# HKUST-KnowComp/DummyNode4GraphLearning

Hardware: AMD Instinct MI355X
Metric: edges/sec fwd+bwd on dummy-augmented RGIN conv (higher is better)
Workload: dtype bf16; 1 GPU; config5: RGINLayer(256,256,R=16,basis,relu) fwd+bwd, ONE global batch of 32768 graphs cut by parallel.shard_graphs over 1 GPU(s) (rank 0: N=1015808, E=3997696), SI dummy augmentation; global_edges=3997696, parallelism=dp1, rows_P=3112960, grad_bucket_bytes=2491904, hip_graph=True, sub_batches=1

## Files before the change

dummynode4graphlearning_amd/_lib.py:

```python
import ctypes
import os

import torch

_HERE = os.path.dirname(os.path.abspath(__file__))
LIB_PATH = os.environ.get("DN_HIP_LIB") or os.path.join(_HERE, "libdn_hip.so")

c_i32, c_i64, c_f32, c_sz = ctypes.c_int32, ctypes.c_int64, ctypes.c_float, ctypes.c_size_t
P = ctypes.c_void_p

class WgradJob(ctypes.Structure):
    _fields_ = [("A", P), ("A2", P), ("idx_a", P), ("G", P), ("G2", P), ("idx_g", P), ("mask_a_bits", P), ("na1", c_i32), ("ng1", c_i32),
                ("colsum_of", c_i32), ("first_rel", c_i32), ("row0", c_i32), ("act_slope", c_f32)]


class BatchCol(ctypes.Structure):
    _fields_ = [("src", P), ("dst", P), ("row_bytes", c_i32), ("level", c_i32), ("rebase", c_i32), ("int_width", c_i32),
                ("src_global", c_i32), ("ptr_tail", c_i32)]


_SIGS = {
    "dn_version": (ctypes.c_int, []),
    "dn_last_error": (ctypes.c_char_p, []),
    "dn_runtime_probe": (ctypes.c_int, [P]),
# ... 41 lines not shown
                                                P, P, P]),
    "dn_layer_graphs_bwd_bf16": (ctypes.c_int, [P, c_i32, P, P, c_i32, P, P, c_f32, P, P, P, P, P, P, P, c_i64, c_i64, P, P, P, P, P, P, P,
                                                P]),
    "dn_conv_graphs_max_nodes": (c_i32, []),
    "dn_conv_graphs_max_edges": (c_i32, []),
    "dn_conv_graphs_bf16": (ctypes.c_int, [P, c_i32, P, c_i32, P, P, c_i32, P, P, P, P, P, c_i64, c_i64, P, P, P, P, P, P]),
    "dn_conv_index_workspace_bytes": (c_sz, [c_i64, c_i64, c_i64, c_i64, c_i32, c_i64]),
    "dn_conv_index_build_i32": (ctypes.c_int, [c_i64, c_i64, c_i64, c_i64, P, P, P, P, P, c_i32, c_f32] + [P] * 10 +
                                [ctypes.POINTER(c_i64), ctypes.POINTER(c_i32), ctypes.POINTER(c_i32),
                                 ctypes.POINTER(c_i32), P, P, P, P, P, ctypes.POINTER(c_i32)] +
                                [c_i32, c_i32, c_i64] + [P] * 8 + [c_i32, c_i64] + [P] * 8 + [c_i32, c_i32, P, P] + [c_i32, c_i32, c_i64, P, P] +
                                [ctypes.POINTER(c_i32), P, c_sz, P]),
    "dn_row_tables_build_i32": (ctypes.c_int, [c_i32, P, c_i32, c_i64, P, P, ctypes.c_uint64, P]),
    "dn_sweep_tables_build_i32": (ctypes.c_int, [c_i32, P, P, P, c_i64, c_i32, c_i32, ctypes.c_uint64, P, P, P]),
    "dn_slot_table_build_i32": (ctypes.c_int, [c_i64, c_i32, c_i32, P, P, c_i32, c_i32, P, P, P, P]),
    "dn_fold_tables_build_async_i32": (ctypes.c_int, [c_i64, c_i64, P, P, P, P, P, P, c_sz, P]),
    "dn_rows_wgrad_workspace_bytes": (c_sz, [c_i64, c_i32, c_i32]),
    "dn_rows_wgrad_bf16": (ctypes.c_int, [P, P, c_i32, P, P, P, c_i32, P, c_i32, c_i32, c_i64, P, c_i64, P, P, c_i32,
                                          c_i32, P, P, P, P, P, c_f32, P, c_sz, P]),
    "dn_rows_transform_bf16": (ctypes.c_int, [P, P, c_i32, P, c_i32, c_i32, P, P, c_i32, P, P, c_i64, P, c_i32, c_f32, P]),
    "dn_relu_bwd_bf16": (ctypes.c_int, [P, P, P, c_i64, c_f32, P]),
    "dn_rows_chain2_bf16": (ctypes.c_int, [P, c_i32, P, P, c_i32, P, P, P, P, c_i32, c_i64, P, P, P, P, c_i32, c_f32, P]),
    "dn_mlp_bwd_fused_bf16": (ctypes.c_int, [P, P, P, P, P, c_i64, c_i32, P, c_i64, P, P, c_i32, P, P, P, c_f32, P, c_sz, P]),
    "dn_rows_selfsum_bf16": (ctypes.c_int, [P, c_i32, P, P, P, P, c_i32, P, c_i32, c_i64, P, P, P, c_i32, P, P, c_i32, c_i32, c_i32, P]),
    "dn_overflow_rows_add_bf16": (ctypes.c_int, [P, c_i32, P, c_i32, c_i64, P, P, c_i32, c_i32, c_i32, P, P]),
    "dn_close_units_capacity": (c_i64, [c_i64, c_i64, c_i32]),
    "dn_close_units_workspace_bytes": (c_sz, [c_i64, c_i32]),
    "dn_close_units_build_i32": (ctypes.c_int, [c_i64, c_i32, c_i32, P, c_i64, c_i32, c_i32, P, P, c_i64, c_i32, c_i32, P, P, P, c_i64, P,
                                                P, P, P, c_i32, P, c_sz, P]),
    "dn_fold_graph_tiles_build_i32": (ctypes.c_int, [c_i64, c_i64, P, P, P, P, P, P, P]),
    "dn_fold_graph_tiles_multi_capacity": (c_i64, [c_i64, c_i32]),
    "dn_fold_graph_tiles_multi_build_i32": (ctypes.c_int, [c_i64, c_i64, P, P, P, c_i32, P, P, P, P, c_i64, P, P]),
    "dn_rows_close_bf16": (ctypes.c_int, [P, c_i32, P, c_i32, P, P, P, P, c_i32, P, P, c_i64, P, P, P, P, P, P, P]),
    "dn_bdd_compose": (ctypes.c_int, [P, c_i64, c_i32, c_i32, c_i32, c_i32, P, P]),
    "dn_bdd_extract": (ctypes.c_int, [P, c_i64, c_i32, c_i32, c_i32, c_i32, P, P]),
    "dn_fold_tables_workspace_bytes": (c_sz, [c_i64]),
    "dn_fold_tables_build_i32": (ctypes.c_int, [c_i64, c_i64, P, P, P, P, ctypes.POINTER(ctypes.c_int32), P, c_sz, P]),
    "dn_fold_tail_bf16": (ctypes.c_int, [P, P, c_i64, c_i32, P, P, P, P, c_i32, P]),
    "dn_rows_transform_f32": (ctypes.c_int, [P, P, c_i32, P, c_i32, c_i32, P, P, c_i32, P, P, c_i64, P, c_i32, c_f32, P, c_i32, c_i32, c_i32, P]),
    "dn_rows_wgrad_f32": (ctypes.c_int, [P, P, c_i32, P, P, P, c_i32, P, c_i32, c_i32, c_i64, P, c_i64, P, P, c_i32, P, P, P,
                                         c_i32, c_f32, P, c_sz, P]),
    "dn_relu_bwd_f32": (ctypes.c_int, [P, P, P, c_i64, c_f32, P]),
    "dn_rows_gemm_f32": (ctypes.c_int, [P, P, P, c_i32, c_i32, c_i32, P, c_i64, P, P]),
    "dn_rows_gemm_bf16": (ctypes.c_int, [P, P, P, c_i32, c_i32, c_i32, P, c_i64, P, P]),
    "dn_rows_wgrad_any_workspace_bytes": (c_sz, [c_i64, c_i32, c_i32]),
    "dn_rows_wgrad_any_f32": (ctypes.c_int, [P, P, c_i32, c_i32, c_i64, P, c_i64, P, P, P, P, c_sz, P]),
# ... 138 lines not shown
```

dummynode4graphlearning_amd/csrc/build.py:

```python
import hashlib
import os
import subprocess
import sys
from concurrent.futures import ThreadPoolExecutor

HERE = os.path.dirname(os.path.abspath(__file__))
PKG = os.path.dirname(HERE)
ROOT = os.path.dirname(PKG)
SOURCES = ["dn_runtime.hip", "dn_segment.hip", "dn_index.hip", "dn_index_local.hip", "dn_conv_index.hip", "dn_graphsum.hip", "dn_rel.hip", "dn_rel_ring.hip", "dn_close.hip", "dn_conv_graph.hip", "dn_chain2.hip", "dn_mlp_bwd.hip", "dn_weights.hip", "dn_rel_f32.hip", "dn_gemm.hip", "dn_norm.hip", "dn_simodel.hip", "dn_dual.hip", "dn_batch.hip", "dn_lrp.hip", "dn_hgt.hip"]
HEADERS = ["dn_common.h", "dn_internal.h", os.path.join(ROOT, "include", "dn_hip.h")]
LIB = os.path.join(PKG, "libdn_hip.so")
OBJDIR = os.path.join(HERE, "_obj")
ARCH = "gfx950"
FLAGS = ["-O3", "-std=c++17", "-fPIC", "--offload-arch=" + ARCH, "-fno-gpu-rdc", "-Wno-unused-result",
         "-I" + os.path.join(ROOT, "include")]


def _hipcc():
    for c in (os.environ.get("HIPCC"), "/opt/rocm/bin/hipcc", "hipcc"):
        if c and (os.path.isabs(c) and os.path.exists(c) or not os.path.isabs(c)):
            return c
    raise RuntimeError("hipcc not found")


def _digest(paths):
    h = hashlib.sha256()
    for p in paths:
        with open(p, "rb") as f:
            h.update(f.read())
    h.update(" ".join(FLAGS).encode())
    return h.hexdigest()

# ... 47 lines not shown
```

dummynode4graphlearning_amd/csrc/dn_internal.h:

```cpp
#pragma once
#include <hip/hip_runtime.h>
#include <stdint.h>

namespace dn_internal {

int launch_transform_ring256(const void* X, const void* X2, int32_t n1, const int32_t* idx, const void* Wn, const void* bias,
                             int32_t relu, int32_t nt_store, const void* mask_pos, const int32_t* tiles, int64_t num_tiles,
                             int64_t tiles_per_wg, void* Y, int32_t w_kn, float slope, hipStream_t st);

bool chain2_ring_supported(bool has_mask0, bool has_mask1, bool has_bits1, bool has_bits2);
int launch_chain2_ring256(const void* X, const void* W1n, const void* b1, const void* W2n, const void* b2, int32_t flags,
                          const void* mask0, const void* mask1, int64_t N, void* Y1, void* Y2, void* bits1, void* bits2,
                          float slope, hipStream_t st);

int launch_wgrad_reduce(const float* workspace, const int32_t* chunk_ptr, int64_t num_chunks, int32_t H, int64_t R, void* out,
                        int32_t out_is_f32, bool with_colsum, float* out_colsum, void* out_colsum_lp, hipStream_t st);

constexpr int kRilPlanWords = 14;

int ril_queue(int64_t G, int64_t N, int64_t R, int64_t E, const int32_t* node_ptr, const int32_t* edge_ptr, const int32_t* src,
              const int32_t* dst, const int32_t* etype, int32_t self_loop, float edge_frac, int32_t* row_in, int32_t* row_out,
              int32_t* aux_f_ptr, int32_t* aux_f_idx, int32_t* aux_b_ptr, int32_t* aux_b_idx, int32_t* dst_ptr, int32_t* dst_rows,
              int32_t* src_ptr, int32_t* src_rows, int32_t* rel_ptr_dev, int32_t* tile_ptr_f, int32_t* fold_info_f,
              int32_t* tile_ptr_b, int32_t* fold_info_b, bool verdicts, bool plan, void* workspace, size_t workspace_bytes,
              int32_t** meta_dev, hipStream_t st);
void ril_unpack(const int32_t* h_meta, int64_t R, int64_t* host_counts, int32_t* host_rel_ptr, int32_t* host_modes,
                int32_t* host_status, int32_t* host_absorb);

struct CloseUnitsDir {
    const int32_t *tile_ptr, *list_ptr, *list_rows;
    int32_t num_edge_rows, drop_beg, drop_end;
// ... 24 lines not shown
```

dummynode4graphlearning_amd/csrc/dn_rel_ring.hip:

```cpp
#include "dn_common.h"
#include "dn_internal.h"

namespace {

typedef __bf16 bf16_t;
typedef bf16_t bf16x8 __attribute__((ext_vector_type(8)));
typedef float f32x4 __attribute__((ext_vector_type(4)));
typedef unsigned int u32x4 __attribute__((ext_vector_type(4)));

struct Tile {
    int32_t rel, beg, end, pad;
};

constexpr int kH = 256;
constexpr int kRowB = 2 * kH;
constexpr int kTR = 32;
constexpr int kStageB = kTR * kRowB;
constexpr int kNS = 8;
constexpr int kCompute = 8, kLoaders = 4;
constexpr int kThreads = 64 * (kCompute + kLoaders);
constexpr int kRowsPerLoader = kTR / kLoaders;
constexpr int kDmaPerTile = kRowsPerLoader / 2;
constexpr int kBatch = 8;
constexpr int kRecRing = 32, kIdxRing = 16, kDescRing = 32;

__device__ __forceinline__ uint32_t pack_bf16x2(float a, float b) {
    typedef bf16_t bf16x2 __attribute__((ext_vector_type(2)));
    bf16x2 v;
    v[0] = (bf16_t)a;
    v[1] = (bf16_t)b;
    return __builtin_bit_cast(uint32_t, v);
}

#ifdef DN_RING_STATS
__device__ unsigned long long g_ring_stats[256][10];
#define DN_STAMP() __builtin_amdgcn_s_memtime()
#define DN_STAT(var, expr) var += (expr)
#else
#define DN_STAMP() 0ull
#define DN_STAT(var, expr)
#endif

__device__ int32_t g_zero_idx[64];

#define DN_DS_READ128(dst, addr, OFF) asm volatile("ds_read_b128 %0, %1 offset:" #OFF : "=v"(dst) : "v"(addr))

template <bool MASK, bool IDX, bool EPI, bool HASX2>
__global__ __launch_bounds__(kThreads) void rows_transform_ring_kernel(
    const bf16_t* __restrict__ X, const bf16_t* __restrict__ X2, int32_t n1, const int32_t* __restrict__ idx,
    const bf16_t* __restrict__ Wn, const bf16_t* __restrict__ bias, int32_t flags, const bf16_t* __restrict__ mask_pos,
    const Tile* __restrict__ tiles, int32_t num_tiles, int32_t tiles_per_wg, bf16_t* __restrict__ Y, float slope) {
    __shared__ __attribute__((aligned(1024))) char lds[kNS * kStageB];
    __shared__ __attribute__((aligned(16))) int32_t descL[kDescRing][4];
    __shared__ __attribute__((aligned(128))) int32_t recR[kLoaders][kRecRing][4];
    __shared__ __attribute__((aligned(256))) int32_t idxR[kLoaders][kIdxRing][kRowsPerLoader];
    __shared__ __attribute__((aligned(16))) char wscr[kCompute][2048];
    typedef __attribute__((address_space(3))) char* lds_wp;
    const unsigned lds_base = (unsigned)(uintptr_t)(lds_wp)lds;
    const unsigned desc_base = (unsigned)(uintptr_t)(lds_wp)&descL[0][0];
    const int tid = threadIdx.x, lane = tid & 63;
    const int wave = __builtin_amdgcn_readfirstlane(tid >> 6);
    const int t_beg = (int)blockIdx.x * tiles_per_wg;
    int nt = min(t_beg + tiles_per_wg, num_tiles) - t_beg;
    if (nt <= 0) return;
    tiles += t_beg;
#ifdef DN_TUNING_ENV
    if (nt <= 512 && !(flags & (128 << 3))) {
#else
    if (nt <= 512) {
#endif
        bool live[8];
#pragma unroll
        for (int c = 0; c < 8; ++c) {
            const int k = 64 * c + lane;
// ... 51 lines not shown
        auto prep = [&](int u, const char* (&src)[kDmaPerTile]) {
            typedef int32_t i32x4 __attribute__((ext_vector_type(4)));
            const i32x4 iv = *reinterpret_cast<const i32x4*>(&idxR[q][u % kIdxRing][4 * rin]);
#pragma unroll
            for (int j = 0; j < kDmaPerTile; ++j) {
                int32_t r = iv[j];
#ifdef DN_TUNING_ENV
                if (flags & 16) r &= 1023;
#endif
                const char* base = reinterpret_cast<const char*>(X) + (size_t)r * kRowB;
                if constexpr (HASX2)
                    if (r >= n1) base = reinterpret_cast<const char*>(X2) + (size_t)(r - n1) * kRowB;
                src[j] = base + swoff[j];
            }
        };
        auto rows = [&](int u, const char* (&src)[kDmaPerTile]) {
            const unsigned st = lds_base + (unsigned)(u % kNS) * kStageB + (unsigned)(kRowsPerLoader * q) * kRowB;
#ifdef DN_TUNING_ENV
            if (flags & 128) return;
#endif
#pragma unroll
            for (int j = 0; j < kDmaPerTile; ++j) glds16(src[j], st + (unsigned)(2 * j) * kRowB);
        };
        auto batch = [&](int u) {
            if ((u & (kBatch - 1)) == 0) {
                stage_idx(u + kBatch);
                dma_recs(u + 2 * kBatch);
            }
        };
        dma_recs(0);
        dma_recs(kBatch);
        wait_vmcnt<0>();
        stage_idx(0);
        wait_vmcnt<0>();
#pragma unroll 1
        for (int u = 0; u < kNS - 2; ++u) {
            batch(u);
            prep(u, srcA);
            rows(u, srcA);
        }
        batch(kNS - 2);
        prep(kNS - 2, srcA);
        batch(kNS - 1);
        prep(kNS - 1, srcB);
        wait_vmcnt<kDmaPerTile*(kNS - 3)>();
        asm volatile("s_waitcnt lgkmcnt(0)" ::: "memory");
        __builtin_amdgcn_s_barrier();
        unsigned long long st_vm = 0, st_bar = 0, st_body = 0;
        const unsigned long long l0 = DN_STAMP();
#pragma unroll 1
        for (int t = 0; t < nt; t += 2) {
            const unsigned long long a0 = DN_STAMP();
#ifdef DN_TUNING_ENV
            if (flags & 128) wait_vmcnt<0>();
#endif
            wait_vmcnt<kDmaPerTile*(kNS - 5)>();
            asm volatile("s_waitcnt lgkmcnt(0)" ::: "memory");
            const unsigned long long a1 = DN_STAMP();
            __builtin_amdgcn_s_barrier();
            const unsigned long long a2 = DN_STAMP();
            rows(t + kNS - 2, srcA);
            rows(t + kNS - 1, srcB);
            batch(t + kNS);
            prep(t + kNS, srcA);
            prep(t + kNS + 1, srcB);
            DN_STAT(st_vm, a1 - a0); DN_STAT(st_bar, a2 - a1); DN_STAT(st_body, DN_STAMP() - a2);
        }
        wait_vmcnt<0>();
#ifdef DN_RING_STATS
        if (q == 0 && lane == 0 && blockIdx.x < 256) {
            g_ring_stats[blockIdx.x][4] = DN_STAMP() - l0; g_ring_stats[blockIdx.x][5] = st_vm;
            g_ring_stats[blockIdx.x][6] = st_bar; g_ring_stats[blockIdx.x][7] = st_body;
        }
#endif
        return;
    }

    const bool relu = (flags & 1) != 0, nt_store = (flags & 2) != 0;
#ifdef DN_TUNING_ENV
    if ((flags & 1024)) __builtin_amdgcn_s_setprio(2);
#endif
    const int n0 = 32 * wave;
    const int j = lane & 15, g = lane >> 4;
    const unsigned off0 = lds_base + (unsigned)(j * kRowB + ((g ^ j) << 4));
    const int colA0 = 8 * (j >> 2) + (j & 3);
    const size_t ocol = (size_t)(n0 + 8 * g);
    bf16x8 wf[8][2];
    u32x4 bv = {0u, 0u, 0u, 0u};
// ... 186 lines not shown
#endif
}
#undef DN_DS_READ128

}

namespace dn_internal {

int launch_transform_ring256(const void* X_, const void* X2, int32_t n1, const int32_t* idx, const void* Wn, const void* bias,
                             int32_t relu, int32_t nt_store, const void* mask_pos, const int32_t* tiles, int64_t num_tiles,
                             int64_t tiles_per_wg, void* Y, int32_t w_kn, float slope, hipStream_t st) {
#ifdef DN_TUNING_ENV
    if (tiles_per_wg <= 0 && dn_knob("DN_TF_RING_WGS", 0) > 0)
        tiles_per_wg = dn_cdiv(num_tiles, dn_knob("DN_TF_RING_WGS", 0));
#endif
    if (tiles_per_wg <= 0) tiles_per_wg = dn_cdiv(num_tiles, 256);
    const int64_t grid = dn_cdiv(num_tiles, tiles_per_wg);
    const int abl = dn_knob("DN_TF_ABL", 0);
    if (dn_knob("DN_TF_NT", 1) == 0) nt_store = 0;
    const int32_t flags = (relu ? 1 : 0) | (nt_store ? 2 : 0) | (w_kn ? 4 : 0) | ((abl & 255) << 3);
#define DN_RING_LAUNCH(M, I, E, X)                                                                                      \
    hipLaunchKernelGGL((rows_transform_ring_kernel<M, I, E, X>), dim3((unsigned)grid), dim3(kThreads), 0, st, (const bf16_t*)X_, \
                       (const bf16_t*)X2, n1, idx, (const bf16_t*)Wn, (const bf16_t*)bias, flags, (const bf16_t*)mask_pos,      \
                       reinterpret_cast<const Tile*>(tiles), (int32_t)num_tiles, (int32_t)tiles_per_wg, (bf16_t*)Y, slope)
    const bool epi = bias != nullptr || relu != 0;
    const bool x2 = X2 != nullptr;
    if (mask_pos) {
        if (idx) DN_RING_LAUNCH(true, true, true, true);
        else DN_RING_LAUNCH(true, false, true, false);
    } else if (idx) {
        if (!epi && !x2) DN_RING_LAUNCH(false, true, false, false);
        else if (!epi) DN_RING_LAUNCH(false, true, false, true);
        else DN_RING_LAUNCH(false, true, true, true);
    } else {
        if (!epi) DN_RING_LAUNCH(false, false, false, false);
        else DN_RING_LAUNCH(false, false, true, false);
    }
#undef DN_RING_LAUNCH
    DN_CHECK_LAUNCH();
    return DN_OK;
}

}

#ifdef DN_RING_STATS
extern "C" int dn_debug_ring_stats(unsigned long long* out) {
    return hipMemcpyFromSymbol(out, HIP_SYMBOL(g_ring_stats), sizeof(g_ring_stats)) == hipSuccess ? 0 : -2;
}
#endif
```

dummynode4graphlearning_amd/ops.py:

```python
import ctypes
import os as _os
import threading as _threading
from typing import NamedTuple

import torch

from . import _lib
from ._lib import check, lib, ptr, require_gpu, stream_ptr

I32 = torch.int32


class KernelTimer:

    def __init__(self):
        self.records = []
        self.enabled = True

    def launch(self, tag, fn):
        if not self.enabled:
            return fn()
        a, b = torch.cuda.Event(enable_timing=True), torch.cuda.Event(enable_timing=True)
        a.record()
        r = fn()
# ... 1521 lines not shown
            ix._units[d] = build_close_units(*lists, N, P, drop=drop, tile_ptr=info.graph_tiles[0], agg=True, multi=info.multi)
        else:
            if info is not None and info.fold_info is None:
                _late_fold_tables(ix, d, info)
            ix._units[d] = build_close_units(*lists, N, P, drop=drop)


def _closing_tables(ix, kind="slots"):
    if kind == "slots" and not ix._slots:
        _build_slot_tables(ix)
    elif kind != "slots" and not ix._units:
        _build_unit_streams(ix)


def _close_kind(H, dtype):
    return "units" if (CLOSE_RING_ENABLED and H == 256 and dtype == torch.bfloat16) else "slots"


FOLD_ENABLED = _os.environ.get("DN_FOLD", "1") != "0"


class _Fold:
    __slots__ = ("rel", "beg", "end", "n", "fold_info", "part_ptr", "num_parts", "main_tiles", "sweep_tiles", "add_idx",
                 "graph_tiles", "multi")

    def __init__(self, ix, direction, cand):
        self.rel, self.beg, self.end, self.n = cand
        self.fold_info = self.part_ptr = self.graph_tiles = self.multi = None
        self.num_parts = int(2 * self.n + ix.num_nodes // 32 + 1)
        self.main_tiles = None
        self.sweep_tiles = None
        self.add_idx = _fold_add_idx(ix, direction, cand)


def _row_index_fold(ix, direction, kind="slots"):
    _closing_tables(ix, kind)
    return ix._fold[direction]


class RowIndexSet:

    def __init__(self, src=None, dst=None, etype=None, num_nodes=None, num_rels=None, self_loop=None, node_ptr=None, edge_ptr=None,
                 closing_hint=None, index=None):
        self.index = ix = index if index is not None else RowIndex(
            src, dst, etype, int(num_nodes), num_rels, self_loop=self_loop, node_ptr=node_ptr, edge_ptr=edge_ptr, closing_hint=closing_hint)
        self.num_nodes, self.num_rels, self.self_loop = ix.num_nodes, ix.num_rels, ix.self_loop
        self.parts = [(0, ix.num_nodes, ix)]
        self.max_rows = self.num_rows = ix.num_rows
        self.num_all_rels = ix.num_all_rels
        self._ybuf = {}

# ... 614 lines not shown

    @staticmethod
    @_backward_in_forward_mode
    def backward(ctx, gout):
        iset, slope = ctx.index_set, ctx.slope
        ix = iset.index
        x, h, h1, bits1, bits2, W, W_loop, w1, w2, aux = ctx.saved_tensors
        g = gout.contiguous()
        H, R = 256, W.shape[0]
        g1, g0 = rows_chain2(g, w2, None, False, w1, None, False, mask0_bits=bits2, mask1_bits=bits1, w_kn=(True, True), slope=slope)
        gx = torch.empty_like(x)
        aux_b = message_pass(g0, PassWeights(W, W_loop, kn=False), None, ix, "b", iset.ybuf(H, g.dtype, g.device), gx)
        grads = layer_wgrad(ix, "wide", H, W.dtype, ctx.has,
                            dict(A=x, A2=aux if ctx.has[3] else None, G=g0, G2=aux_b, colsum_of=2 | ((R + 1) << 8)),
                            dict(A=g1, G=h), dict(A=g, G=h1, mask_a_bits=bits2, slope=slope))
        return (gx if ctx.needs_input_grad[0] else None, None, None, *grads)


def rgin_layer_wide(x, W, W_loop, bias, linears, slope, index_set):
    return _RginLayerWideFn.apply(x, float(slope), index_set, W, W_loop, bias, linears[0].weight, linears[0].bias,
                                  linears[1].weight, linears[1].bias)


LAYER_F32_ENABLED = _os.environ.get("DN_LAYER_F32", "1") != "0"
CHAIN2_F32_ENABLED = _os.environ.get("DN_CHAIN2_F32", "1") != "0"


def rgin_layer_f32_ok(x, W, W_loop, bias, linears, index_set):
    if not (LAYER_F32_ENABLED and W_loop is not None and len(linears) == 2 and not f32_mode()):
        return False
    H = x.shape[1] if x.dim() == 2 else 0
    ok = lambda t: t is None or (t.is_cuda and t.dtype == torch.float32)
    return (x.is_cuda and x.dtype == torch.float32 and H in (64, 128) and x.shape[0] > 0 and tuple(W.shape[1:]) == (H, H)
            and W.dtype == x.dtype and tuple(W_loop.shape) == (H, H) and ok(W_loop) and ok(bias)
            and all(ok(l.weight) and ok(l.bias) and tuple(l.weight.shape) == (H, H) for l in linears)
            and index_set.index.num_rows > 0 and _kn_ok(x))


class _RginLayerF32Fn(torch.autograd.Function):

    @staticmethod
    def forward(ctx, x, slope, index_set, W, W_loop, bias, w1, b1, w2, b2, residual=False):
        ctx.f32_mode = f32_mode()
        x = x.contiguous()
        ix = index_set.index
        N, H = x.shape
# ... 1307 lines not shown
```

dummynode4graphlearning_amd/subgraph_isomorphism/rgin.py:

```python
import torch as th
import torch.nn as nn

from .. import ops
from .act import map_activation_str_to_layer
from .init import init_weight

NODEFEAT, EDGETYPE, NODEOUTPUT = "node_feat", "edge_type", "node_out"


def _fused_slope(act):
    if isinstance(act, nn.ReLU):
        return 0.0
    if isinstance(act, nn.LeakyReLU):
        return float(act.negative_slope)
    return None


def dense_relation_weights(layer):
    if layer.regularizer in ("none", "basis"):
        if layer.num_bases < layer.num_rels:
            w = layer.weight.view(layer.num_bases, layer.input_dim * layer.hidden_dim)
            return th.matmul(layer.w_comp, w).view(layer.num_rels, layer.input_dim, layer.hidden_dim)
        return layer.weight
    si, so = layer.input_dim // layer.num_bases, layer.hidden_dim // layer.num_bases
# ... 106 lines not shown
            if self.bias is not None:
                out = out + self.bias
        if len(self.mlp) > 0:
            out, act_done = self._run_mlp(out)
        else:
            out, act_done = self.act(out), False
        if not act_done:
            out = self.act(out)
        out = self.drop(out)
        return out, edge_type

    def _small_layer(self, node_feat, W, index, residual=False):
        if not self.self_loop:
            return None
        mods = list(self.mlp)
        linears = [m for m in mods if isinstance(m, nn.Linear)]
        slope = _fused_slope(self.act)
        if slope is None or len(mods) != 3 or not all(isinstance(m, nn.Linear) or _fused_slope(m) == slope for m in mods):
            return None
        if ops.rgin_layer_small_ok(node_feat, W, self.loop_weight, self.bias, linears, index):
            return ops.rgin_layer_small(node_feat, W, self.loop_weight, self.bias, linears, slope, index)
        if ops.rgin_layer_wide_ok(node_feat, W, self.loop_weight, self.bias, linears, index):
            return ops.rgin_layer_wide(node_feat, W, self.loop_weight, self.bias, linears, slope, index)
        if ops.rgin_layer_f32_ok(node_feat, W, self.loop_weight, self.bias, linears, index):
            self._residual_done = bool(residual)
            return ops.rgin_layer_f32(node_feat, W, self.loop_weight, self.bias, linears, slope, index, residual=residual)
        return None

    def _run_mlp(self, out):
        mods = list(self.mlp)
        linears = [m for m in mods if isinstance(m, nn.Linear)]
        slope = _fused_slope(self.act)
        if (slope is not None and all(isinstance(m, nn.Linear) or _fused_slope(m) == slope for m in mods)
                and ops.relu_mlp_supported(out, linears)):
            return ops.relu_mlp(out, linears, slope), True
        i, act_done = 0, False
        while i < len(mods):
            m = mods[i]
            if isinstance(m, nn.Linear):
                nxt = mods[i + 1] if i + 1 < len(mods) else self.act
                fuse = isinstance(nxt, nn.ReLU)
                out = ops.linear_act(out, m.weight, m.bias, relu=fuse)
                if fuse:
                    if i + 1 < len(mods):
                        i += 1
                    else:
# ... 72 lines not shown
```

include/dn_hip.h:

```cpp
#ifndef DN_HIP_H
#define DN_HIP_H

#include <stddef.h>
#include <stdint.h>

#ifdef __cplusplus
extern "C" {
#endif

#define DN_OK 0
#define DN_ERR_ARG (-1)
#define DN_ERR_HIP (-2)
#define DN_ERR_WORKSPACE (-3)
#define DN_ERR_UNSUPPORTED (-4)

typedef void* dn_stream_t;

int dn_version(void);
const char* dn_last_error(void);
int dn_runtime_probe(const void* device_ptr);

int dn_gather_segsum_f32(const float* in, int64_t in_rows, int32_t H, const int32_t* idx,
                         const float* scale, const int32_t* ptr, int64_t S, int64_t M, float* out,
                         const float* self_in, float self_coef, int32_t mean, dn_stream_t stream);
// ... 390 lines not shown
                             int64_t Q, int32_t* col_rows, int64_t* col_cnt, dn_stream_t stream);
int32_t dn_lrp_stage_bytes(void);
int32_t dn_lrp_pair_nodes(void);
int dn_lrp_pool_fwd_f32(int64_t N, int64_t E, int32_t H, int32_t L, const int32_t* uptr, const int32_t* unbr, const int32_t* ueid,
                        const int32_t* upos, const int32_t* ego, const int64_t* count, const float* t_node, const float* t_edge,
                        const float* bias, const float* factor, int32_t pool_mean, int32_t act_on, float slope, float* pooled,
                        float* out, dn_stream_t stream);
int dn_lrp_pool_bwd_f32(int64_t N, int64_t E, int32_t H, int32_t L, const int32_t* uptr, const int32_t* unbr, const int32_t* ueid,
                        const int32_t* upos, const int32_t* ego, const int64_t* count, const float* t_node, const float* t_edge,
                        const float* bias, const float* factor, int32_t pool_mean, int32_t act_on, float slope, const float* pooled,
                        const float* g, float* d_tnode, float* d_tedge, float* d_bias, float* d_factor, dn_stream_t stream);

int dn_hgt_attn_fwd_f32(int64_t N, int64_t E, int64_t P, int32_t H, int32_t heads, const int32_t* dst_ptr, const int32_t* pair_ptr,
                        const int32_t* pair_row, const int32_t* src_s, const int32_t* et_s, const int32_t* row_s, const float* Qp,
                        const float* K, const float* V, const float* pri, float scale, float* att, float* U, dn_stream_t stream);
int dn_hgt_attn_bwd_dst_f32(int64_t N, int64_t E, int64_t P, int32_t H, int32_t heads, const int32_t* dst_ptr, const int32_t* pair_ptr,
                            const int32_t* pair_rel, const int32_t* pair_row, const int32_t* src_s, const int32_t* row_s, const float* Qp,
                            const float* K, const float* V, const float* pri, float scale, const float* att, const float* dU, float* dl,
                            float* dQp, float* dpri_part, dn_stream_t stream);
int dn_hgt_attn_bwd_src_f32(int64_t N, int64_t E, int64_t P, int32_t H, int32_t heads, const int32_t* out_ptr, const int32_t* out_pos,
                            const int32_t* out_row, const float* Qp, const float* dU, const float* att, const float* dl, float* dK,
                            float* dV, dn_stream_t stream);

#ifdef __cplusplus
}
#endif
#endif
```

Before: 1.367 billion edges/s.

## Add chained RGIN layer path that folds first MLP weight grads into relation wgrad

Result: faster. 1.390 billion edges/s (median of 6 runs) (+1.7%).

```diff
diff --git a/dummynode4graphlearning_amd/_lib.py b/dummynode4graphlearning_amd/_lib.py
--- a/dummynode4graphlearning_amd/_lib.py
+++ b/dummynode4graphlearning_amd/_lib.py
@@ -87,6 +87,9 @@
     "dn_relu_bwd_bf16": (ctypes.c_int, [P, P, P, c_i64, c_f32, P]),
     "dn_rows_chain2_bf16": (ctypes.c_int, [P, c_i32, P, P, c_i32, P, P, P, P, c_i32, c_i64, P, P, P, P, c_i32, c_f32, P]),
     "dn_mlp_bwd_fused_bf16": (ctypes.c_int, [P, P, P, P, P, c_i64, c_i32, P, c_i64, P, P, c_i32, P, P, P, c_f32, P, c_sz, P]),
+    "dn_layer_chain_dgrad_bf16": (ctypes.c_int, [P, P, c_i64, c_i32, P, c_i64, P, P, P]),
+    "dn_layer_chain_wgrad_combine_workspace_bytes": (c_sz, [c_i64, c_i32]),
+    "dn_layer_chain_wgrad_combine": (ctypes.c_int, [P, P, P, P, P, P, c_i64, c_i32, P, P, P, P, P, c_sz, P]),
     "dn_rows_selfsum_bf16": (ctypes.c_int, [P, c_i32, P, P, P, P, c_i32, P, c_i32, c_i64, P, P, P, c_i32, P, P, c_i32, c_i32, c_i32, P]),
     "dn_overflow_rows_add_bf16": (ctypes.c_int, [P, c_i32, P, c_i32, c_i64, P, P, c_i32, c_i32, c_i32, P, P]),
     "dn_close_units_capacity": (c_i64, [c_i64, c_i64, c_i32]),
diff --git a/dummynode4graphlearning_amd/csrc/build.py b/dummynode4graphlearning_amd/csrc/build.py
--- a/dummynode4graphlearning_amd/csrc/build.py
+++ b/dummynode4graphlearning_amd/csrc/build.py
@@ -7,7 +7,7 @@
 HERE = os.path.dirname(os.path.abspath(__file__))
 PKG = os.path.dirname(HERE)
 ROOT = os.path.dirname(PKG)
-SOURCES = ["dn_runtime.hip", "dn_segment.hip", "dn_index.hip", "dn_index_local.hip", "dn_conv_index.hip", "dn_graphsum.hip", "dn_rel.hip", "dn_rel_ring.hip", "dn_close.hip", "dn_conv_graph.hip", "dn_chain2.hip", "dn_mlp_bwd.hip", "dn_weights.hip", "dn_rel_f32.hip", "dn_gemm.hip", "dn_norm.hip", "dn_simodel.hip", "dn_dual.hip", "dn_batch.hip", "dn_lrp.hip", "dn_hgt.hip"]
+SOURCES = ["dn_runtime.hip", "dn_segment.hip", "dn_index.hip", "dn_index_local.hip", "dn_conv_index.hip", "dn_graphsum.hip", "dn_rel.hip", "dn_rel_ring.hip", "dn_close.hip", "dn_conv_graph.hip", "dn_chain2.hip", "dn_mlp_bwd.hip", "dn_chain_wgrad.hip", "dn_weights.hip", "dn_rel_f32.hip", "dn_gemm.hip", "dn_norm.hip", "dn_simodel.hip", "dn_dual.hip", "dn_batch.hip", "dn_lrp.hip", "dn_hgt.hip"]
 HEADERS = ["dn_common.h", "dn_internal.h", os.path.join(ROOT, "include", "dn_hip.h")]
 LIB = os.path.join(PKG, "libdn_hip.so")
 OBJDIR = os.path.join(HERE, "_obj")
diff --git a/dummynode4graphlearning_amd/csrc/dn_chain_wgrad.hip b/dummynode4graphlearning_amd/csrc/dn_chain_wgrad.hip
--- /dev/null
+++ b/dummynode4graphlearning_amd/csrc/dn_chain_wgrad.hip
@@ -0,0 +1,142 @@
+#include "dn_common.h"
+#include "dn_internal.h"
+#include "../../include/dn_hip.h"
+
+namespace {
+
+typedef __bf16 bf16_t;
+
+constexpr int kH = 256;
+constexpr int kTile = 64;
+constexpr int kKC = 32;
+constexpr int kThreads = 256;
+constexpr int kAld = kTile + 2;
+
+__device__ __forceinline__ double bf16_to_f64(bf16_t v) { return (double)(float)v; }
+
+__device__ __forceinline__ bf16_t f64_to_bf16(double d) {
+    float f = (float)d;
+    if ((double)f != d && f == f && fabsf(f) < __builtin_huge_valf()) {
+        uint32_t u = __float_as_uint(f);
+        if (fabs((double)f) > fabs(d)) u -= 1u;
+        f = __uint_as_float(u | 1u);
+    }
+    return (bf16_t)f;
+}
+
+__global__ __launch_bounds__(kThreads) void chain_combine_products_kernel(const float* __restrict__ M, const bf16_t* __restrict__ W1,
+                                                                          const bf16_t* __restrict__ Wc,
+                                                                          const bf16_t* __restrict__ Wc_loop, int32_t R,
+                                                                          bf16_t* __restrict__ dWc, double* __restrict__ part) {
+    __shared__ __attribute__((aligned(16))) double As[kKC * kAld];
+    __shared__ __attribute__((aligned(16))) double Bs[kKC * kTile];
+    const int tid = threadIdx.x, ty = tid >> 4, tx = tid & 15;
+    const int m0 = (int)(blockIdx.x >> 2) * kTile, n0 = (int)(blockIdx.x & 3) * kTile;
+    const int r = (int)blockIdx.y, kind = (int)blockIdx.z;
+    const float* Mr = M + (size_t)r * kH * kH;
+    const bf16_t* B = kind == 0 ? W1 : (r < R ? Wc + (size_t)r * kH * kH : Wc_loop);
+    double acc[4][4];
+#pragma unroll
+    for (int i = 0; i < 4; ++i)
+#pragma unroll
+        for (int j = 0; j < 4; ++j) acc[i][j] = 0.0;
+    float ra[8];
+    bf16_t rb[8];
+    auto fetch = [&](int kc) __attribute__((always_inline)) {
+#pragma unroll
+        for (int s = 0; s < 8; ++s) {
+            if (kind == 0) ra[s] = Mr[(size_t)(m0 + (tid >> 5) + 8 * s) * kH + kc + (tid & 31)];
+            else ra[s] = Mr[(size_t)(kc + (tid >> 6) + 4 * s) * kH + m0 + (tid & 63)];
+            rb[s] = B[(size_t)(kc + (tid >> 6) + 4 * s) * kH + n0 + (tid & 63)];
+        }
+    };
+    fetch(0);
+    for (int kc = 0; kc < kH; kc += kKC) {
+#pragma unroll
+        for (int s = 0; s < 8; ++s) {
+            if (kind == 0) As[(tid & 31) * kAld + (tid >> 5) + 8 * s] = (double)ra[s];
+            else As[((tid >> 6) + 4 * s) * kAld + (tid & 63)] = (double)ra[s];
+            Bs[((tid >> 6) + 4 * s) * kTile + (tid & 63)] = bf16_to_f64(rb[s]);
+        }
+        if (kc + kKC < kH) fetch(kc + kKC);
+        __syncthreads();
+#pragma unroll 8
+        for (int k = 0; k < kKC; ++k) {
+            const double2 a01 = *reinterpret_cast<const double2*>(&As[k * kAld + 4 * ty]);
+            const double2 a23 = *reinterpret_cast<const double2*>(&As[k * kAld + 4 * ty + 2]);
+            const double2 b01 = *reinterpret_cast<const double2*>(&Bs[k * kTile + 4 * tx]);
+            const double2 b23 = *reinterpret_cast<const double2*>(&Bs[k * kTile + 4 * tx + 2]);
+            const double a[4] = {a01.x, a01.y, a23.x, a23.y}, b[4] = {b01.x, b01.y, b23.x, b23.y};
+#pragma unroll
+            for (int i = 0; i < 4; ++i)
+#pragma unroll
+                for (int j = 0; j < 4; ++j) acc[i][j] = fma(a[i], b[j], acc[i][j]);
+        }
+        __syncthreads();
+    }
+#pragma unroll
+    for (int i = 0; i < 4; ++i)
+#pragma unroll
+        for (int j = 0; j < 4; ++j) {
+            const size_t o = (size_t)r * kH * kH + (size_t)(m0 + 4 * ty + i) * kH + n0 + 4 * tx + j;
+            if (kind == 0) dWc[o] = f64_to_bf16(acc[i][j]);
+            else part[o] = acc[i][j];
+        }
+}
+
+__global__ __launch_bounds__(kH) void chain_combine_finish_kernel(const double* __restrict__ part, const float* __restrict__ c,
+                                                                  const bf16_t* __restrict__ W1, const bf16_t* __restrict__ bias,
+                                                                  int32_t R, bf16_t* __restrict__ dW1, bf16_t* __restrict__ db,
+                                                                  bf16_t* __restrict__ db1) {
+    const int h = threadIdx.x, j = (int)blockIdx.x;
+    if (j < kH) {
+        double sum = 0.0;
+        for (int r = 0; r <= R; ++r) sum += part[(size_t)r * kH * kH + (size_t)j * kH + h];
+        if (bias) sum = fma((double)c[j], bf16_to_f64(bias[h]), sum);
+        dW1[(size_t)j * kH + h] = f64_to_bf16(sum);
+        return;
+    }
+    if (db) {
+        double sum = 0.0;
+        for (int jj = 0; jj < kH; ++jj) sum = fma((double)c[jj], bf16_to_f64(W1[(size_t)jj * kH + h]), sum);
+        db[h] = f64_to_bf16(sum);
+    }
+    if (db1) db1[h] = (bf16_t)c[h];
+}
+
+}
+
+extern "C" int dn_layer_chain_dgrad_bf16(const void* G1, const void* W_kn, int64_t N, int32_t H, const int32_t* tiles, int64_t num_tiles,
+                                         void* G0, void* seg_sums, dn_stream_t stream) {
+    DN_REQUIRE(H == 256, "dn_layer_chain_dgrad: unsupported width %d (256 only)", H);
+    DN_REQUIRE(N >= 0 && N < 0x7fffffffLL && num_tiles >= 0 && num_tiles < 0x7fffffffLL, "dn_layer_chain_dgrad: bad sizes");
+    if (num_tiles == 0) return DN_OK;
+    DN_REQUIRE(G1 && W_kn && tiles && G0 && seg_sums, "dn_layer_chain_dgrad: NULL pointer");
+    DN_REQUIRE((reinterpret_cast<uintptr_t>(G1) | reinterpret_cast<uintptr_t>(W_kn) | reinterpret_cast<uintptr_t>(tiles) |
+                reinterpret_cast<uintptr_t>(G0) | reinterpret_cast<uintptr_t>(seg_sums)) % 16 == 0, "dn_layer_chain_dgrad: unaligned pointer");
+    return dn_internal::launch_transform_ring256_seg(G1, W_kn, tiles, num_tiles, G0, seg_sums, (hipStream_t)stream);
+}
+
+extern "C" size_t dn_layer_chain_wgrad_combine_workspace_bytes(int64_t R, int32_t H) {
+    return R >= 0 && H > 0 ? (size_t)(R + 1) * (size_t)H * (size_t)H * sizeof(double) : 0;
+}
+
+extern "C" int dn_layer_chain_wgrad_combine(const float* M, const float* c, const void* W1, const void* Wc, const void* Wc_loop,
+                                            const void* bias, int64_t R, int32_t H, void* dWc, void* db, void* dW1, void* db1,
+                                            void* workspace, size_t workspace_bytes, dn_stream_t stream) {
+    DN_REQUIRE(H == 256, "dn_layer_chain_wgrad_combine: unsupported width %d (256 only)", H);
+    DN_REQUIRE(R >= 0 && R < 65535, "dn_layer_chain_wgrad_combine: bad relation count");
+    DN_REQUIRE(M && c && W1 && Wc_loop && dWc && dW1 && workspace && (Wc || R == 0), "dn_layer_chain_wgrad_combine: NULL pointer");
+    DN_REQUIRE(workspace_bytes >= dn_layer_chain_wgrad_combine_workspace_bytes(R, H), "dn_layer_chain_wgrad_combine: workspace too small");
+    DN_REQUIRE((reinterpret_cast<uintptr_t>(M) | reinterpret_cast<uintptr_t>(workspace)) % 16 == 0,
+               "dn_layer_chain_wgrad_combine: unaligned pointer");
+    hipStream_t st = (hipStream_t)stream;
+    double* part = (double*)workspace;
+    hipLaunchKernelGGL(chain_combine_products_kernel, dim3((kH / kTile) * (kH / kTile), (unsigned)(R + 1), 2), dim3(kThreads), 0, st, M,
+                       (const bf16_t*)W1, (const bf16_t*)Wc, (const bf16_t*)Wc_loop, (int32_t)R, (bf16_t*)dWc, part);
+    DN_CHECK_LAUNCH();
+    hipLaunchKernelGGL(chain_combine_finish_kernel, dim3(kH + 1), dim3(kH), 0, st, (const double*)part, c, (const bf16_t*)W1,
+                       (const bf16_t*)bias, (int32_t)R, (bf16_t*)dW1, (bf16_t*)db, (bf16_t*)db1);
+    DN_CHECK_LAUNCH();
+    return DN_OK;
+}
diff --git a/dummynode4graphlearning_amd/csrc/dn_internal.h b/dummynode4graphlearning_amd/csrc/dn_internal.h
--- a/dummynode4graphlearning_amd/csrc/dn_internal.h
+++ b/dummynode4graphlearning_amd/csrc/dn_internal.h
@@ -7,6 +7,9 @@
 int launch_transform_ring256(const void* X, const void* X2, int32_t n1, const int32_t* idx, const void* Wn, const void* bias,
                              int32_t relu, int32_t nt_store, const void* mask_pos, const int32_t* tiles, int64_t num_tiles,
                              int64_t tiles_per_wg, void* Y, int32_t w_kn, float slope, hipStream_t st);
+
+int launch_transform_ring256_seg(const void* X, const void* W_kn, const int32_t* tiles, int64_t num_tiles, void* Y, void* seg_sums,
+                                 hipStream_t st);
 
 bool chain2_ring_supported(bool has_mask0, bool has_mask1, bool has_bits1, bool has_bits2);
 int launch_chain2_ring256(const void* X, const void* W1n, const void* b1, const void* W2n, const void* b2, int32_t flags,
diff --git a/dummynode4graphlearning_amd/csrc/dn_rel_ring.hip b/dummynode4graphlearning_amd/csrc/dn_rel_ring.hip
--- a/dummynode4graphlearning_amd/csrc/dn_rel_ring.hip
+++ b/dummynode4graphlearning_amd/csrc/dn_rel_ring.hip
@@ -45,11 +45,12 @@
 
 #define DN_DS_READ128(dst, addr, OFF) asm volatile("ds_read_b128 %0, %1 offset:" #OFF : "=v"(dst) : "v"(addr))
 
-template <bool MASK, bool IDX, bool EPI, bool HASX2>
+template <bool MASK, bool IDX, bool EPI, bool HASX2, bool SEG = false>
 __global__ __launch_bounds__(kThreads) void rows_transform_ring_kernel(
     const bf16_t* __restrict__ X, const bf16_t* __restrict__ X2, int32_t n1, const int32_t* __restrict__ idx,
     const bf16_t* __restrict__ Wn, const bf16_t* __restrict__ bias, int32_t flags, const bf16_t* __restrict__ mask_pos,
-    const Tile* __restrict__ tiles, int32_t num_tiles, int32_t tiles_per_wg, bf16_t* __restrict__ Y, float slope) {
+    const Tile* __restrict__ tiles, int32_t num_tiles, int32_t tiles_per_wg, bf16_t* __restrict__ Y, float slope,
+    bf16_t* __restrict__ seg_out) {
     __shared__ __attribute__((aligned(1024))) char lds[kNS * kStageB];
     __shared__ __attribute__((aligned(16))) int32_t descL[kDescRing][4];
     __shared__ __attribute__((aligned(128))) int32_t recR[kLoaders][kRecRing][4];
@@ -147,6 +148,28 @@
 #pragma unroll
             for (int j = 0; j < kDmaPerTile; ++j) glds16(src[j], st + (unsigned)(2 * j) * kRowB);
         };
+        auto seg_sum = [&](int u) {
+            const int32_t* rp = &recR[q][u % kRecRing][0];
+            const int rows_u = __builtin_amdgcn_readfirstlane(min(max(rp[2] - rp[1], 0), kTR));
+            const int sg = __builtin_amdgcn_readfirstlane(rp[3]);
+            const int s0 = sg & 0xff, s1 = min((sg >> 8) & 0xff, rows_u);
+            const char* stg = lds + (u % kNS) * kStageB + (lane & 7) * 2;
+            const int p = 8 * q + (lane >> 3);
+            float acc = 0.f;
+#pragma unroll 1
+            for (int r = s0; r < s1; r += 8) {
+                uint32_t v[8];
+#pragma unroll
+                for (int k = 0; k < 8; ++k) {
+                    const int rr = min(r + k, kTR - 1);
+                    v[k] = *reinterpret_cast<const uint16_t*>(stg + rr * kRowB + ((p ^ (rr & 15)) << 4));
+                }
+#pragma unroll
+                for (int k = 0; k < 8; ++k)
+                    if (r + k < s1) acc += __uint_as_float(v[k] << 16);
+            }
+            seg_out[(size_t)(t_beg + u) * kH + 64 * q + lane] = (bf16_t)acc;
+        };
         auto batch = [&](int u) {
             if ((u & (kBatch - 1)) == 0) {
                 stage_idx(u + kBatch);
@@ -189,6 +212,10 @@
             batch(t + kNS);
             prep(t + kNS, srcA);
             prep(t + kNS + 1, srcB);
+            if constexpr (SEG) {
+                seg_sum(t);
+                if (t + 1 < nt) seg_sum(t + 1);
+            }
             DN_STAT(st_vm, a1 - a0); DN_STAT(st_bar, a2 - a1); DN_STAT(st_body, DN_STAMP() - a2);
         }
         wait_vmcnt<0>();
@@ -421,7 +448,8 @@
 #define DN_RING_LAUNCH(M, I, E, X)                                                                                      \
     hipLaunchKernelGGL((rows_transform_ring_kernel<M, I, E, X>), dim3((unsigned)grid), dim3(kThreads), 0, st, (const bf16_t*)X_, \
                        (const bf16_t*)X2, n1, idx, (const bf16_t*)Wn, (const bf16_t*)bias, flags, (const bf16_t*)mask_pos,      \
-                       reinterpret_cast<const Tile*>(tiles), (int32_t)num_tiles, (int32_t)tiles_per_wg, (bf16_t*)Y, slope)
+                       reinterpret_cast<const Tile*>(tiles), (int32_t)num_tiles, (int32_t)tiles_per_wg, (bf16_t*)Y, slope,      \
+                       (bf16_t*)nullptr)
     const bool epi = bias != nullptr || relu != 0;
     const bool x2 = X2 != nullptr;
     if (mask_pos) {
@@ -440,6 +468,19 @@
     return DN_OK;
 }
 
+int launch_transform_ring256_seg(const void* X, const void* W_kn, const int32_t* tiles, int64_t num_tiles, void* Y, void* seg_sums,
+                                 hipStream_t st) {
+    const int64_t tiles_per_wg = dn_cdiv(num_tiles, 256);
+    const int64_t grid = dn_cdiv(num_tiles, tiles_per_wg);
+    const int32_t flags = 2 | 4;
+    hipLaunchKernelGGL((rows_transform_ring_kernel<false, false, false, false, true>), dim3((unsigned)grid), dim3(kThreads), 0, st,
+                       (const bf16_t*)X, (const bf16_t*)nullptr, 0x7fffffff, (const int32_t*)nullptr, (const bf16_t*)W_kn,
+                       (const bf16_t*)nullptr, flags, (const bf16_t*)nullptr, reinterpret_cast<const Tile*>(tiles), (int32_t)num_tiles,
+                       (int32_t)tiles_per_wg, (bf16_t*)Y, 0.f, (bf16_t*)seg_sums);
+    DN_CHECK_LAUNCH();
+    return DN_OK;
+}
+
 }
 
 #ifdef DN_RING_STATS
diff --git a/dummynode4graphlearning_amd/ops.py b/dummynode4graphlearning_amd/ops.py
--- a/dummynode4graphlearning_amd/ops.py
+++ b/dummynode4graphlearning_amd/ops.py
@@ -1567,11 +1567,11 @@
 
 class _Fold:
     __slots__ = ("rel", "beg", "end", "n", "fold_info", "part_ptr", "num_parts", "main_tiles", "sweep_tiles", "add_idx",
-                 "graph_tiles", "multi")
+                 "graph_tiles", "multi", "seg_tiles")
 
     def __init__(self, ix, direction, cand):
         self.rel, self.beg, self.end, self.n = cand
-        self.fold_info = self.part_ptr = self.graph_tiles = self.multi = None
+        self.fold_info = self.part_ptr = self.graph_tiles = self.multi = self.seg_tiles = None
         self.num_parts = int(2 * self.n + ix.num_nodes // 32 + 1)
         self.main_tiles = None
         self.sweep_tiles = None
@@ -2232,6 +2232,118 @@
                                   linears[1].weight, linears[1].bias)
 
 
+LAYER_CHAIN_WGRAD_ENABLED = _os.environ.get("DN_LAYER_CHAIN_WGRAD", "1") != "0"
+
+
+def _chain_seg_tiles(ix, fold):
+    if fold.seg_tiles is None:
+        n, v = fold.n, ix.dirs["b"]
+        tp, ap = fold.graph_tiles[0][:n + 1], v.aux_ptr[:n + 1]
+        beg, end = tp[:n], tp[1:]
+        s0 = v.aux_idx[ap[:n].long()] - beg
+        seg = s0 | ((s0 + (ap[1:] - ap[:n])) << 8)
+        fold.seg_tiles = torch.stack([torch.zeros_like(beg), beg, end, seg], 1).to(I32).contiguous()
+    return fold.seg_tiles
+
+
+def layer_chain_dgrad(g1, w1, seg_tiles):
+    g1, w1 = g1.contiguous(), w1.contiguous()
+    require_gpu(g1, w1, seg_tiles)
+    N, H = g1.shape
+    T = int(seg_tiles.shape[0])
+    assert g1.dtype == torch.bfloat16 and w1.dtype == g1.dtype and H == 256 and tuple(w1.shape) == (H, H)
+    assert seg_tiles.dtype == I32 and seg_tiles.dim() == 2 and seg_tiles.shape[1] == 4 and seg_tiles.is_contiguous()
+    g0 = torch.empty_like(g1)
+    sums = torch.empty((T, H), dtype=g1.dtype, device=g1.device)
+
+    def _launch():
+        check(lib().dn_layer_chain_dgrad_bf16(ptr(g1), ptr(w1), N, H, ptr(seg_tiles), T, ptr(g0), ptr(sums), stream_ptr()),
+              "dn_layer_chain_dgrad_bf16")
+    launch_tagged("chain_dgrad", _launch)
+    return g0, sums
+
+
+def layer_chain_wgrad_combine(M, c, w1, W, W_loop, bias):
+    M, c, w1, W, W_loop = M.contiguous(), c.contiguous(), w1.contiguous(), W.contiguous(), W_loop.contiguous()
+    require_gpu(M, c, w1, W, W_loop, bias)
+    R, H = W.shape[0], 256
+    assert M.dtype == torch.float32 and tuple(M.shape) == (R + 1, H, H) and c.dtype == torch.float32 and c.numel() == H
+    assert w1.dtype == torch.bfloat16 and tuple(w1.shape) == (H, H) and W.dtype == w1.dtype and tuple(W.shape[1:]) == (H, H)
+    assert W_loop.dtype == w1.dtype and tuple(W_loop.shape) == (H, H)
+    assert bias is None or (bias.dtype == w1.dtype and bias.numel() == H and bias.is_contiguous())
+    dev = M.device
+    dWc = torch.empty((R + 1, H, H), dtype=w1.dtype, device=dev)
+    dW1 = torch.empty((H, H), dtype=w1.dtype, device=dev)
+    db = torch.empty((H,), dtype=w1.dtype, device=dev) if bias is not None else None
+    db1 = torch.empty((H,), dtype=w1.dtype, device=dev)
+    ws = _ws(lib().dn_layer_chain_wgrad_combine_workspace_bytes(R, H), dev)
+
+    def _launch():
+        check(lib().dn_layer_chain_wgrad_combine(ptr(M), ptr(c), ptr(w1), ptr(W), ptr(W_loop), ptr(bias), R, H, ptr(dWc), ptr(db), ptr(dW1),
+                                                 ptr(db1), ptr(ws), ws.numel(), stream_ptr()), "dn_layer_chain_wgrad_combine")
+    launch_tagged("chain_combine", _launch)
+    return dWc, db, dW1, db1
+
+
+def rgin_layer_chain_ok(x, W, W_loop, bias, linears, index_set):
+    if not (LAYER_CHAIN_WGRAD_ENABLED and MLP_BWD_FUSED_ENABLED and CHAIN2_ENABLED and W_loop is not None and bias is not None
+            and len(linears) == 2 and all(l.bias is not None for l in linears)):
+        return False
+    if not (x.is_cuda and x.dtype == torch.bfloat16 and x.dim() == 2 and x.shape[1] == 256 and W.dtype == x.dtype
+            and tuple(W.shape[1:]) == (256, 256) and tuple(W_loop.shape) == (256, 256) and W_loop.dtype == x.dtype
+            and bias.dtype == x.dtype and x.requires_grad and torch.is_grad_enabled()
+            and all(l.weight.dtype == x.dtype and l.bias.dtype == x.dtype and tuple(l.weight.shape) == (256, 256) for l in linears)):
+        return False
+    ix = index_set.index
+    N = x.shape[0]
+    if not (_selfsum_ok(ix, x) and _kn_ok(x) and N >= max(MLP_BWD_FUSED_MIN_ROWS, 1) and ix.num_rows + 2 * N > WIDE_LAYER_MAX_ROWS
+            and _close_kind(256, x.dtype) == "units" and not conv_graphs_ok(x, PassWeights(W, W_loop, kn=True), ix)):
+        return False
+    for d in ("f", "b"):
+        fold = _row_index_fold(ix, d, "units")
+        if fold is None or fold.graph_tiles is None or fold.multi is not None or not ix.close_units(d).agg:
+            return False
+    return ix.dirs["b"].n_aux == ix._fold["b"].n
+
+
+class _RginLayerChainFn(torch.autograd.Function):
+
+    @staticmethod
+    def forward(ctx, x, slope, index_set, W, W_loop, bias, w1, b1, w2, b2):
+        ctx.f32_mode = f32_mode()
+        x = x.contiguous()
+        ix = index_set.index
+        h = torch.empty_like(x)
+        aux = message_pass(x, PassWeights(W, W_loop, kn=True), bias, ix, "f", index_set.ybuf(256, x.dtype, x.device), h)
+        h1, h2, bits1, bits2 = rows_chain2(h, w1, b1, True, w2, b2, True, want_bits=True, slope=float(slope))
+        ctx.index_set, ctx.slope = index_set, float(slope)
+        ctx.save_for_backward(x, h1, bits1, bits2, W, W_loop, bias, w1, w2, aux if aux is not None else x.new_empty(0))
+        return h2
+
+    @staticmethod
+    @_backward_in_forward_mode
+    def backward(ctx, gout):
+        iset, slope = ctx.index_set, ctx.slope
+        ix = iset.index
+        x, h1, bits1, bits2, W, W_loop, bias, w1, w2, aux = ctx.saved_tensors
+        g = gout.contiguous()
+        H, R = 256, W.shape[0]
+        _, chunks = _dense_table(x.shape[0], x.device)
+        gw2, gb2, g1 = mlp_bwd_fused(g, h1, w2, chunks, mask_in_bits=bits2, mask_out_bits=bits1, slope=slope)
+        g0, g1_sums = layer_chain_dgrad(g1, w1, _chain_seg_tiles(ix, ix._fold["b"]))
+        gx = torch.empty_like(x)
+        message_pass(g0, PassWeights(W, W_loop, kn=False), None, ix, "b", iset.ybuf(H, g.dtype, g.device), gx)
+        M, cs = rows_wgrad(x, g1, ix.chunk_table, R + 1, idx_a=ix.row_in, idx_g=ix.row_out, A2=aux if ix.num_aux_f else None,
+                           G2=g1_sums, out_dtype=torch.float32, colsum_of=2, colsum_rel=R)
+        gAll, gb, gw1, gb1 = layer_chain_wgrad_combine(M, cs[R], w1, W, W_loop, bias)
+        return (gx, None, None, gAll[:R], gAll[R], gb, gw1, gb1, gw2, gb2.to(g.dtype))
+
+
+def rgin_layer_chain(x, W, W_loop, bias, linears, slope, index_set):
+    return _RginLayerChainFn.apply(x, float(slope), index_set, W, W_loop, bias, linears[0].weight, linears[0].bias,
+                                   linears[1].weight, linears[1].bias)
+
+
 LAYER_F32_ENABLED = _os.environ.get("DN_LAYER_F32", "1") != "0"
 CHAIN2_F32_ENABLED = _os.environ.get("DN_CHAIN2_F32", "1") != "0"
 
diff --git a/dummynode4graphlearning_amd/subgraph_isomorphism/rgin.py b/dummynode4graphlearning_amd/subgraph_isomorphism/rgin.py
--- a/dummynode4graphlearning_amd/subgraph_isomorphism/rgin.py
+++ b/dummynode4graphlearning_amd/subgraph_isomorphism/rgin.py
@@ -152,6 +152,8 @@
             return ops.rgin_layer_small(node_feat, W, self.loop_weight, self.bias, linears, slope, index)
         if ops.rgin_layer_wide_ok(node_feat, W, self.loop_weight, self.bias, linears, index):
             return ops.rgin_layer_wide(node_feat, W, self.loop_weight, self.bias, linears, slope, index)
+        if ops.rgin_layer_chain_ok(node_feat, W, self.loop_weight, self.bias, linears, index):
+            return ops.rgin_layer_chain(node_feat, W, self.loop_weight, self.bias, linears, slope, index)
         if ops.rgin_layer_f32_ok(node_feat, W, self.loop_weight, self.bias, linears, index):
             self._residual_done = bool(residual)
             return ops.rgin_layer_f32(node_feat, W, self.loop_weight, self.bias, linears, slope, index, residual=residual)
diff --git a/include/dn_hip.h b/include/dn_hip.h
--- a/include/dn_hip.h
+++ b/include/dn_hip.h
@@ -436,6 +436,13 @@
                             const int32_t* out_row, const float* Qp, const float* dU, const float* att, const float* dl, float* dK,
                             float* dV, dn_stream_t stream);
 
+int dn_layer_chain_dgrad_bf16(const void* G1, const void* W_kn, int64_t N, int32_t H, const int32_t* tiles, int64_t num_tiles, void* G0,
+                              void* seg_sums, dn_stream_t stream);
+size_t dn_layer_chain_wgrad_combine_workspace_bytes(int64_t R, int32_t H);
+int dn_layer_chain_wgrad_combine(const float* M, const float* c, const void* W1, const void* Wc, const void* Wc_loop, const void* bias,
+                                 int64_t R, int32_t H, void* dWc, void* db, void* dW1, void* db1, void* workspace,
+                                 size_t workspace_bytes, dn_stream_t stream);
+
 #ifdef __cplusplus
 }
 #endif
```
